# imperatormk/candle-birefnet

Hardware: AMD Instinct MI355X
Metric: images/sec @1024x1024 Swin-L (higher is better)
Workload: dtype f32 storage+accumulate; GEMM operands as two fp16 planes of the power-of-two-scaled operand (22-bit mantissa), 3 fp16 MFMAs/product (fp32-equivalent inside the fp16 range: |GEMM input| < 8190); 1 GPU; BASELINE configs[1]: Swin-L 1024x1024 batch=1 fp32 on 1xMI355X (single-image latency); batch_per_gpu=1, global_batch=1, size=1024, deform_mode=reference_cpu, compute=f32_half2, streams_per_gpu=1, branch_streams_per_gpu=5, inputs=resident in HBM (torch cuda tensors), weights: synthetic seed 42

## Files before the change

### candle_birefnet_amd/csrc/kernels/gemm_split.hip

```cpp
#include "../brn_kernels.h"
#include "gemm_common.h"
#include "gemm_split_stages.h"

namespace brn {

constexpr int SPLIT_LD = 40;

template <int BM, int BN, int WM, int WN, int MODE, int NP, bool H = false>
__global__ void __launch_bounds__(WM* WN * 64) gemm_split_kernel(const GemmParams p) {
    static_assert(!H || NP == 2, "fp16 planes come in pairs");
    constexpr int SLD = SPLIT_LD;
    constexpr int NT = WM * WN * 64;
    constexpr int RPP = NT / 8;
    constexpr int PA = BM / RPP;
    constexpr int WRPP = NT / 4;
    constexpr int PB = BN / WRPP;
    constexpr int WTM = BM / WM, WTN = BN / WN, TM = WTM / 32, TN = WTN / 32;
    static_assert(PA >= 1 && PB >= 1 && TM >= 1 && TN >= 1, "tile too small for the thread count");

    constexpr int SMEM_MAIN = NP * (BM + BN) * SLD * 2, SMEM_EPI = WM * WN * EPI_WAVE_FLOATS * 4;
    __shared__ __attribute__((aligned(16))) char smem_raw[SMEM_MAIN > SMEM_EPI ? SMEM_MAIN : SMEM_EPI];
    __bf16* smem = reinterpret_cast<__bf16*>(smem_raw);
    __bf16* As = smem;
    __bf16* Bs = smem + NP * BM * SLD;

    const int tid = threadIdx.x, lane = tid & 63, wave = tid >> 6;
    const int wm = wave / WN, wn = wave % WN;
    const TileSlice ts = tile_slice<BM, BN>(p, BK);
    const int slice = ts.slice, m0 = ts.m0, n0 = ts.n0, kt0 = ts.kt0, nk = ts.nk;

    const int kq = tid & 7, lrow = tid >> 3;
    long a_base[PA];
    int a_iy[PA], a_ix[PA];
    bool a_ok[PA];
#pragma unroll
    for (int i = 0; i < PA; ++i) gather_row_init<MODE>(p, m0 + lrow + i * RPP, a_ok[i], a_base[i], a_iy[i], a_ix[i]);
    const int wc = tid & 3, wrow = tid >> 2;
    const long wrow_stride = (long)p.K * NP;
    const __bf16* wsrc = reinterpret_cast<const __bf16*>(p.Wp) + (long)(n0 + wrow) * wrow_stride + wc * 8;

    f32x4 ra[2][PA];
    bf16x8 rb[2][NP][PB];
    unsigned am[2][PA];
    constexpr bool DEFORM = MODE == GEMM_DEFORM_NHWC;
    f32x4 rc[DEFORM ? PA : 1][4];
    int rk = 0;
    DeformLoader<PA, 8> dl;
    if constexpr (DEFORM) dl.init(p, m0, lrow, RPP, kq, lane);

    auto gload = [&](int kt, f32x4 (&qa)[PA], bf16x8 (&qb)[NP][PB], unsigned (&qm)[PA]) {
        const int k0 = kt * BK;
#pragma unroll
        for (int pl = 0; pl < NP; ++pl)
#pragma unroll
            for (int i = 0; i < PB; ++i)
                qb[pl][i] = *reinterpret_cast<const bf16x8*>(wsrc + (long)i * WRPP * wrow_stride + (long)kt * (NP * 32) + pl * 32);
        if constexpr (DEFORM) {
            rk = k0;
            dl.template issue<0, PA>(p, k0, rc);
        } else {
            gather_rows_load<MODE>(&p, k0, kq, a_ok, a_base, a_iy, a_ix, qa, qm);
        }
    };
    auto lds_store = [&](const f32x4 (&qa)[PA], const bf16x8 (&qb)[NP][PB], const unsigned (&qm)[PA]) {
#pragma unroll
        for (int i = 0; i < PA; ++i) {
            auto at = [&](int pl) { return As + (pl * BM + lrow + i * RPP) * SLD + kq * 4; };
            if constexpr (DEFORM) stage_a_row<NP, H>(dl.finish(p, rk, i, rc[i]), 0xffffffffu, false, p.a_scale, at);
            else stage_a_row<NP, H>(qa[i], qm[i], true, p.a_scale, at);
        }
        stage_w_planes<NP, PB>(qb, [&](int pl, int i) { return Bs + (pl * BN + wrow + i * WRPP) * SLD + wc * 8; });
    };

    f32x16 acc[TM][TN];
#pragma unroll
    for (int i = 0; i < TM; ++i)
#pragma unroll
        for (int j = 0; j < TN; ++j)
#pragma unroll
            for (int r = 0; r < 16; ++r) acc[i][j][r] = 0.f;

    const __bf16* a_frag = As + (wm * WTM + (lane & 31)) * SLD + (lane >> 5) * 8;
    const __bf16* b_frag = Bs + (wn * WTN + (lane & 31)) * SLD + (lane >> 5) * 8;

    auto compute = [&]() {
#pragma unroll
        for (int ks = 0; ks < 2; ++ks) {
            bf16x8 af[NP][TM], bf[NP][TN];
#pragma unroll
            for (int pl = 0; pl < NP; ++pl) {
#pragma unroll
                for (int i = 0; i < TM; ++i) af[pl][i] = *reinterpret_cast<const bf16x8*>(a_frag + (pl * BM + i * 32) * SLD + ks * 16);
#pragma unroll
                for (int j = 0; j < TN; ++j) bf[pl][j] = *reinterpret_cast<const bf16x8*>(b_frag + (pl * BN + j * 32) * SLD + ks * 16);
            }
            plane_products<NP, H, false>(af, bf, acc);
        }
    };

    if constexpr (DEFORM) {
        if (kt0 < nk) {
            gload(kt0, ra[0], rb[0], am[0]);
            lds_store(ra[0], rb[0], am[0]);
        }
        __syncthreads();
        for (int kt = kt0; kt < nk; ++kt) {
            if (kt + 1 < nk) gload(kt + 1, ra[0], rb[0], am[0]);
            compute();
            __syncthreads();
            if (kt + 1 < nk) {
                lds_store(ra[0], rb[0], am[0]);
                __syncthreads();
            }
        }
    } else {
    if (kt0 < nk) {
        gload(kt0, ra[0], rb[0], am[0]);
        if (kt0 + 1 < nk) gload(kt0 + 1, ra[1], rb[1], am[1]);
        lds_store(ra[0], rb[0], am[0]);
    }
    __syncthreads();
#define BRN_SPLIT_STEP(KT, CUR, NXT)                                  \
    {                                                                 \
        if ((KT) + 2 < nk) gload((KT) + 2, ra[CUR], rb[CUR], am[CUR]);         \
        compute();                                                    \
        __syncthreads();                                              \
        if ((KT) + 1 < nk) {                                          \
            lds_store(ra[NXT], rb[NXT], am[NXT]);            \
            __syncthreads();                                          \
        }                                                             \
    }
    for (int kt = kt0; kt < nk; kt += 2) {
        BRN_SPLIT_STEP(kt, 0, 1)
        if (kt + 1 < nk) BRN_SPLIT_STEP(kt + 1, 1, 0)
    }
#undef BRN_SPLIT_STEP
    }
    gemm_epilogue<TM, TN, WTM, WTN>(p, acc, m0, n0, wm, wn, lane, slice, reinterpret_cast<float*>(smem_raw) + wave * EPI_WAVE_FLOATS);
}

template <int MODE, int NP, int KS, bool DIAG, bool APL, bool H = false>
__global__ void __launch_bounds__(512) __attribute__((amdgpu_waves_per_eu(MODE == GEMM_DEFORM_NHWC && NP == 2 ? 4 : 1)))
gemm_split_ws_kernel(const GemmParams p) {
    using L = WsLayout<NP, KS, APL>;
    constexpr int BM = L::BM, BN = L::BN, WTM = L::WTM, WTN = L::WTN, TM = 2, TN = 2;
    static_assert(!APL || ((NP == 2 || NP == 3) && MODE == GEMM_DENSE), "the P input layout is the NP-plane split of a dense A");
    static_assert(!H || NP == 2, "fp16 planes come in pairs");
    static_assert(L::NBUF == 2, "the producers stage one tile ahead of the consumers; a tile's first fragments are read after the step's barrier");
    constexpr int SLD = L::ROW, KSTEPS = L::KSTEPS, NBUF = L::NBUF, AQ = L::AQ, RPP = L::RPP, PA = L::PA, WQ = L::WQ, WRPP = L::WRPP, PB = L::PB;
    constexpr int APAD = L::APAD, AREG = L::AREG, BUF = L::BUF, EP_LD = L::EP_LD;
    __shared__ __attribute__((aligned(16))) char smem_raw[L::SMEM];
    __bf16* smem = reinterpret_cast<__bf16*>(smem_raw);

    const int tid = threadIdx.x, lane = tid & 63, wave = tid >> 6;
    const int abl = DIAG ? p.abl : 0;
    const bool producer = wave >= 4;
    const TileSlice ts = tile_slice<BM, BN>(p, KS);
    const int slice = ts.slice, m0 = ts.m0, n0 = ts.n0, kt0 = ts.kt0, nk = ts.nk;
    const int nt = nk > kt0 ? nk - kt0 : 0;

    const WsTrace<DIAG> tr(p);
    tr.start(tid);
    f32x16 acc[TM][TN];
    if (producer) {
        const int pt = tid - 256;
        const int kq = pt % AQ, lrow = pt / AQ;
        long a_base[PA];
        int a_iy[PA], a_ix[PA];
        bool a_ok[PA];
        int p_lds[PA];
#pragma unroll
        for (int i = 0; i < PA; ++i) {
            p_lds[i] = 0;
            if (APL) {
                const int q = i * 256 + pt, row = q / (4 * NP), c = q - row * (4 * NP);
                p_lds[i] = ((c >> 2) * BM + row) * SLD + (c >> 2) * APAD + ((c & 3) ^ L::swz_key(row)) * 8;
            }
            gather_row_init<MODE>(p, m0 + lrow + i * RPP, a_ok[i], a_base[i], a_iy[i], a_ix[i]);
        }
        const int wc = pt % WQ, wrow = pt / WQ;
        const int a_sw = ((kq >> 1) ^ L::swz_key(lrow)) * 8 + (kq & 1) * 4;
        const int w_sw = (wc ^ L::swz_key(wrow)) * 8;
        const long wrow_stride = (long)p.K * NP;
        constexpr bool BUFA = MODE == GEMM_DENSE;
        constexpr bool BUFC = MODE == GEMM_CONV_NHWC;
        const int conv_b0 = BUFC ? min(m0, p.M - 1) / (p.Hout * p.Wout) : 0;
        const bool bufc_ok = BUFC && (double)p.Hin * p.Win * p.lda * 8.0 < 2147483648.0;
        __amdgpu_buffer_rsrc_t rsrc_a = BUFC
            ? __builtin_amdgcn_make_buffer_rsrc(const_cast<float*>(p.A + (long)conv_b0 * p.Hin * p.Win * p.lda + p.a_coff), 0, 0x7fffffff, 0x00020000)
            : __builtin_amdgcn_make_buffer_rsrc(const_cast<float*>(p.A + (long)m0 * p.lda), 0, (int)min((long)(p.M - m0) * p.lda * 4, 0x7fffffffL), 0x00020000);
        int conv_pix[PA];
#pragma unroll
        for (int i = 0; i < PA; ++i) {
            conv_pix[i] = 0;
            if (BUFC) {
                const int m = m0 + lrow + i * RPP, hw = p.Hout * p.Wout;
                const int bq = a_ok[i] ? m / hw - conv_b0 : 0;
                conv_pix[i] = (((bq * p.Hin + a_iy[i]) * p.Win + a_ix[i]) * p.lda + kq * 4) * 4;
            }
        }
        __amdgpu_buffer_rsrc_t rsrc_w = __builtin_amdgcn_make_buffer_rsrc(const_cast<__bf16*>(reinterpret_cast<const __bf16*>(p.Wp) + (long)n0 * wrow_stride), 0,
                                                                          0x7fffffff, 0x00020000);
        unsigned voff_a[PA], voff_w[PB];
#pragma unroll
        for (int i = 0; i < PA; ++i) {
            if (APL) { const int q = i * 256 + pt, row = q / (4 * NP), c = q - row * (4 * NP); voff_a[i] = (unsigned)((row * p.lda + c * 4) * 4); }
            else voff_a[i] = (unsigned)(((lrow + i * RPP) * p.lda + kq * 4) * 4);
        }
#pragma unroll
        for (int i = 0; i < PB; ++i) voff_w[i] = (unsigned)(((long)(wrow + i * WRPP) * wrow_stride + wc * 8) * 2);
        f32x4 ra[2][PA];
        bf16x8 rb[2][NP][PB];
        unsigned am[2][PA];
        auto wload = [&](int kt, bf16x8 (&qb)[NP][PB]) {
            const int wk = (KS == 32 ? kt * (NP * 32) : (kt >> 1) * (NP * 32) + (kt & 1) * 16) * 2;
#pragma unroll
            for (int pl = 0; pl < NP; ++pl)
#pragma unroll
                for (int i = 0; i < PB; ++i)
                    qb[pl][i] = __builtin_bit_cast(bf16x8, __builtin_amdgcn_raw_buffer_load_b128(rsrc_w, voff_w[i], wk + pl * 64, 0));
        };
        auto gload = [&](int t, f32x4 (&qa)[PA], bf16x8 (&qb)[NP][PB], unsigned (&qm)[PA]) {
            const int k0 = (kt0 + t) * KS;
            wload(kt0 + t, qb);
            if (BUFA) {
#pragma unroll
                for (int i = 0; i < PA; ++i) {
                    qa[i] = __builtin_bit_cast(f32x4, __builtin_amdgcn_raw_buffer_load_b128(rsrc_a, voff_a[i], APL ? (kt0 + t) * (64 * NP) : k0 * 4, 0));
                    qm[i] = 0xffffffffu;
                }
                return;
            }
            const ConvTap tp = conv_tap(p, k0);
            const int dy = tp.ky * p.dil, dx = tp.kx * p.dil;
            if (bufc_ok) {
                const int tap_off = ((dy * p.Win + dx) * p.lda + tp.ci0) * 4;
#pragma unroll
                for (int i = 0; i < PA; ++i) {
                    const int iy = a_iy[i] + dy, ix = a_ix[i] + dx;
                    const bool ok = a_ok[i] && (unsigned)iy < (unsigned)p.Hin && (unsigned)ix < (unsigned)p.Win;
                    qa[i] = __builtin_bit_cast(f32x4, __builtin_amdgcn_raw_buffer_load_b128(rsrc_a, ok ? (unsigned)(conv_pix[i] + tap_off) : 0x80000000u, 0, 0));
                    qm[i] = 0xffffffffu;
                }
                return;
            }
#pragma unroll
            for (int i = 0; i < PA; ++i) {
                const int iy = a_iy[i] + dy, ix = a_ix[i] + dx;
                const bool ok = a_ok[i] && (unsigned)iy < (unsigned)p.Hin && (unsigned)ix < (unsigned)p.Win;
                const long off = ok ? a_base[i] + ((long)iy * p.Win + ix) * p.lda + tp.ci0 : (long)p.a_coff;
                qa[i] = load4_masked(p.A + off + kq * 4, ok, qm[i]);
            }
        };
        auto w_store = [&](int t, const bf16x8 (&qb)[NP][PB]) {
            __bf16* Bs = smem + (t % NBUF) * BUF + AREG;
            stage_w_planes<NP, PB>(qb, [&](int pl, int i) { return Bs + (pl * BN + wrow + i * WRPP) * SLD + w_sw; });
        };
        auto lds_store = [&](int t, const f32x4 (&qa)[PA], const bf16x8 (&qb)[NP][PB], const unsigned (&qm)[PA]) {
            __bf16* As = smem + (t % NBUF) * BUF;
            if (APL) {
#pragma unroll
                for (int i = 0; i < PA; ++i) {
                    const u32x4 bits = __builtin_bit_cast(u32x4, qa[i]) & qm[i];
                    *reinterpret_cast<u32x4*>(As + p_lds[i]) = bits;
                }
            } else {
#pragma unroll
                for (int i = 0; i < PA; ++i)
                    stage_a_row<NP, H>(qa[i], qm[i], !(BUFA || (BUFC && bufc_ok)), p.a_scale, [&](int pl) { return As + (pl * BM + lrow + i * RPP) * SLD + a_sw; });
            }
            w_store(t, qb);
        };
        if constexpr (MODE == GEMM_DEFORM_NHWC) {
        static_assert(!APL && !DIAG && NBUF == 2 && PA % 2 == 0, "the deformable producer: plain A, the 2-deep ring, rows in two halves");
        constexpr int HR = PA / 2;
        DeformLoader<PA, AQ> dl;
        dl.init(p, m0, lrow, RPP, kq, lane);
        f32x4 rc[PA][4];
        auto a_store = [&](int t, int i, const f32x4 v) {
            __bf16* As = smem + (t % NBUF) * BUF;
            stage_a_row<NP, H>(v, 0xffffffffu, false, p.a_scale, [&](int pl) { return As + (pl * BM + lrow + i * RPP) * SLD + a_sw; });
            __builtin_amdgcn_sched_barrier(0);
        };
        if (nt > 0) { wload(kt0, rb[0]); dl.template issue<0, PA>(p, kt0 * KS, rc); }
        if (nt > 0) {
#pragma unroll
            for (int i = 0; i < PA; ++i) a_store(0, i, dl.finish(p, kt0 * KS, i, rc[i]));
            w_store(0, rb[0]);
        }
        if (nt > 1) { dl.template issue<0, PA>(p, (kt0 + 1) * KS, rc); wload(kt0 + 1, rb[0]); }
        __syncthreads();
        for (int t = 0; t < nt; ++t) {
            const int u = t + 1;
            if (u < nt) {
                const int k0 = (kt0 + u) * KS;
#pragma unroll
                for (int i = 0; i < HR; ++i) a_store(u, i, dl.finish(p, k0, i, rc[i]));
                if (u + 1 < nt) dl.template issue<0, HR>(p, k0 + KS, rc);
#pragma unroll
                for (int i = HR; i < PA; ++i) a_store(u, i, dl.finish(p, k0, i, rc[i]));
                if (u + 1 < nt) dl.template issue<HR, PA>(p, k0 + KS, rc);
                w_store(u, rb[0]);
                if (u + 1 < nt) wload(kt0 + u + 1, rb[0]);
            }
            __syncthreads();
        }
        } else {
        if (nt > 0) gload(0, ra[0], rb[0], am[0]);
        if (nt > 1) gload(1, ra[1], rb[1], am[1]);
        if (nt > 0 && !(abl & 2)) lds_store(0, ra[0], rb[0], am[0]);
        if (nt > 2) gload(2, ra[0], rb[0], am[0]);
        tr.cycles(tid == 256, 8 + 3);
        __syncthreads();
#define BRN_PROD_STEP(T, SET)                                                                      \
        {                                                                                          \
            tr.cycles(tid == 256 && (T) < 24, 16 + (T) * 4 + 0);                                   \
            tr.drain_loads();                                                                      \
            tr.cycles(tid == 256 && (T) < 24, 16 + (T) * 4 + 3);                                   \
            if ((T) + 1 < nt) {                                                                \
                if (!(abl & 2)) lds_store((T) + 1, ra[SET], rb[SET], am[SET]);                 \
                tr.cycles(tid == 256 && (T) < 24, 16 + (T) * 4 + 1);                               \
                if ((T) + 3 < nt && !(abl & 1)) gload((T) + 3, ra[SET], rb[SET], am[SET]); \
            }                                                                                      \
            tr.cycles(tid == 256 && (T) < 24, 16 + (T) * 4 + 2);                                   \
            if (!(abl & 16)) __syncthreads();                                                      \
        }
        for (int t = 0; t < nt; t += 2) {
            BRN_PROD_STEP(t, 1)
            if (t + 1 < nt) BRN_PROD_STEP(t + 1, 0)
        }
#undef BRN_PROD_STEP
        }
        tr.cycles(tid == 256, 8 + 4);
        tr.wall(tid == 256, 8 + 5);
    } else if constexpr (KS == 32 && NP == 2 && !DIAG) {
    f32x4 acc4[4][4];
#pragma unroll
    for (int i = 0; i < 4; ++i)
#pragma unroll
        for (int j = 0; j < 4; ++j) acc4[i][j] = zero4();
    const int wm = wave >> 1, wn = wave & 1;
    const int r16 = lane & 15, kc = lane >> 4;
    const int fch = (kc ^ L::swz_key(r16)) * 8;
    const int a_row = (wm * WTM + r16) * SLD + fch, b_row = AREG + (wn * WTN + r16) * SLD + fch;
    auto read_a = [&](int t, int half, bf16x8 (&af)[NP][2]) {
        const __bf16* buf = smem + (t % NBUF) * BUF;
#pragma unroll
        for (int pl = 0; pl < NP; ++pl)
#pragma unroll
            for (int i = 0; i < 2; ++i) af[pl][i] = *reinterpret_cast<const bf16x8*>(buf + a_row + (pl * BM + (half * 2 + i) * 16) * SLD + pl * APAD);
    };
    auto read_b = [&](int t, int half, bf16x8 (&bf)[NP][2]) {
        const __bf16* buf = smem + (t % NBUF) * BUF;
#pragma unroll
        for (int pl = 0; pl < NP; ++pl)
#pragma unroll
            for (int j = 0; j < 2; ++j) bf[pl][j] = *reinterpret_cast<const bf16x8*>(buf + b_row + (pl * BN + (half * 2 + j) * 16) * SLD);
    };
    bf16x8 fa0[NP][2], fa1[NP][2], fb0[NP][2], fb1[NP][2];
    __syncthreads();
    if (nt > 0) { read_a(0, 0, fa0); read_b(0, 0, fb0); }
    for (int t = 0; t < nt; ++t) {
        read_a(t, 1, fa1);
        read_b(t, 1, fb1);
        plane_products<NP, H, true>(fa0, fb0, acc4, 0, 0);
        plane_products<NP, H, true>(fa1, fb0, acc4, 2, 0);
        plane_products<NP, H, true>(fa0, fb1, acc4, 0, 2);
        plane_products<NP, H, true>(fa1, fb1, acc4, 2, 2);
        __syncthreads();
        if (t + 1 < nt) { read_a(t + 1, 0, fa0); read_b(t + 1, 0, fb0); }
    }
    float* ctile = reinterpret_cast<float*>(smem_raw);
#pragma unroll
    for (int i = 0; i < 4; ++i)
#pragma unroll
        for (int j = 0; j < 4; ++j)
            *reinterpret_cast<f32x4*>(ctile + (wm * WTM + i * 16 + r16) * EP_LD + wn * WTN + j * 16 + 4 * kc) = acc4[i][j];
    } else {
#pragma unroll
    for (int i = 0; i < TM; ++i)
#pragma unroll
        for (int j = 0; j < TN; ++j)
#pragma unroll
            for (int r = 0; r < 16; ++r) acc[i][j][r] = 0.f;
    const int wm = wave >> 1, wn = wave & 1;
    const int fkey = L::swz_key(lane & 31);
    const int a_row = (wm * WTM + (lane & 31)) * SLD, b_row = AREG + (wn * WTN + (lane & 31)) * SLD;
    int f_chunk[KSTEPS];
#pragma unroll
    for (int ks = 0; ks < KSTEPS; ++ks) f_chunk[ks] = (((lane >> 5) + 2 * ks) ^ fkey) * 8;
    auto read_frags = [&](int t, int ks, bf16x8 (&af)[NP][TM], bf16x8 (&bf)[NP][TN]) {
        const __bf16* buf = smem + (t % NBUF) * BUF;
#pragma unroll
        for (int pl = 0; pl < NP; ++pl) {
#pragma unroll
            for (int i = 0; i < TM; ++i) af[pl][i] = *reinterpret_cast<const bf16x8*>(buf + a_row + (pl * BM + i * 32) * SLD + pl * APAD + f_chunk[ks]);
#pragma unroll
            for (int j = 0; j < TN; ++j) bf[pl][j] = *reinterpret_cast<const bf16x8*>(buf + b_row + (pl * BN + j * 32) * SLD + f_chunk[ks]);
        }
    };
    bf16x8 fa0[NP][TM], fb0[NP][TN], fa1[NP][TM], fb1[NP][TN];
    __syncthreads();
    tr.cycles(tid == 0, 3);
    if (nt > 0 && !(abl & 4)) read_frags(0, 0, fa0, fb0);
    for (int t = 0; t < nt; ++t) {
        tr.cycles(tid == 0 && t < 24, 128 + t * 4 + 0);
        if (!(abl & 4)) {
            if (KSTEPS == 2) {
                read_frags(t, 1, fa1, fb1);
                plane_products<NP, H, true>(fa0, fb0, acc);
                plane_products<NP, H, true>(fa1, fb1, acc);
            } else {
                plane_products<NP, H, true>(fa0, fb0, acc);
            }
        }
        tr.cycles(tid == 0 && t < 24, 128 + t * 4 + 1);
        if (!(abl & 16)) __syncthreads();
        if (t + 1 < nt && !(abl & 4)) read_frags(t + 1, 0, fa0, fb0);
    }
    tr.cycles(tid == 0, 4);
    float* ctile = reinterpret_cast<float*>(smem_raw);
    {
        const int row = lane & 31, h4 = (lane >> 5) * 4;
#pragma unroll
        for (int i = 0; i < TM; ++i)
#pragma unroll
            for (int j = 0; j < TN; ++j)
#pragma unroll
                for (int g = 0; g < 4; ++g) {
                    const f32x4 v = {acc[i][j][4 * g], acc[i][j][4 * g + 1], acc[i][j][4 * g + 2], acc[i][j][4 * g + 3]};
                    *reinterpret_cast<f32x4*>(ctile + (wm * WTM + i * 32 + row) * EP_LD + wn * WTN + j * 32 + 8 * g + h4) = v;
                }
    }
    }
    __syncthreads();
    gemm_epilogue_tile<BM, BN, EP_LD>(p, reinterpret_cast<const float*>(smem_raw), m0, n0, tid, slice);
    tr.cycles(tid == 0, 5);
    tr.wall(tid == 0, 6);
}

template <int NP, int KS, bool H>
static hipError_t launch_split_ws_ks(const GemmParams& p, dim3 grid, hipStream_t s) {
    const dim3 block(512);
    if (p.a_planes) {
        if constexpr (NP == 2 && KS == 32) {
            if (p.mode != GEMM_DENSE || p.a_planes != NP) return hipErrorInvalidValue;
#ifdef BRN_DIAG_BUILD
            if constexpr (!H)
                if (p.abl || p.trace) { hipLaunchKernelGGL((gemm_split_ws_kernel<GEMM_DENSE, 2, 32, true, true>), grid, block, 0, s, p); return hipGetLastError(); }
#endif
            hipLaunchKernelGGL((gemm_split_ws_kernel<GEMM_DENSE, 2, 32, false, true, H>), grid, block, 0, s, p);
            return hipGetLastError();
        }
        return hipErrorInvalidValue;
    }
#ifdef BRN_DIAG_BUILD
    if constexpr (!H)
        if (p.mode == GEMM_DENSE && KS == 32 && (p.abl || p.trace)) { hipLaunchKernelGGL((gemm_split_ws_kernel<GEMM_DENSE, NP, 32, true, false>), grid, block, 0, s, p); return hipGetLastError(); }
#endif
    if (p.mode == GEMM_DENSE) hipLaunchKernelGGL((gemm_split_ws_kernel<GEMM_DENSE, NP, KS, false, false, H>), grid, block, 0, s, p);
    else if (p.mode == GEMM_CONV_NHWC) hipLaunchKernelGGL((gemm_split_ws_kernel<GEMM_CONV_NHWC, NP, KS, false, false, H>), grid, block, 0, s, p);
    else if (p.mode == GEMM_DEFORM_NHWC) {
        if constexpr (NP >= 2 && KS == 32) hipLaunchKernelGGL((gemm_split_ws_kernel<GEMM_DEFORM_NHWC, NP, 32, false, false, H>), grid, block, 0, s, p);
        else return hipErrorInvalidValue;
    }
    else return hipErrorInvalidValue;
    return hipGetLastError();
}
template <int NP>
static hipError_t launch_split_ws(const GemmParams& p, hipStream_t s) {
    const int tiles = ((p.M + 127) / 128) * ((p.N + 127) / 128) * p.splitk;
    const dim3 grid(tiles);
    if (p.h2) {
        if constexpr (NP == 2) return launch_split_ws_ks<2, 32, true>(p, grid, s);
        else return hipErrorInvalidValue;
    }
    if constexpr (NP == 3)
        if (tiles > 256 && !(p.abl || p.trace) && p.mode != GEMM_DEFORM_NHWC) return launch_split_ws_ks<3, 16, false>(p, grid, s);
    return launch_split_ws_ks<NP, 32, false>(p, grid, s);
}

template <int BM, int BN, int WM, int WN, int NP, bool H>
static hipError_t launch_split_cfg(const GemmParams& p, hipStream_t s) {
    const int tiles = ((p.M + BM - 1) / BM) * ((p.N + BN - 1) / BN) * p.splitk;
    dim3 grid(tiles), block(WM * WN * 64);
    if (p.mode == GEMM_DENSE) hipLaunchKernelGGL((gemm_split_kernel<BM, BN, WM, WN, GEMM_DENSE, NP, H>), grid, block, 0, s, p);
    else if (p.mode == GEMM_CONV_NHWC) hipLaunchKernelGGL((gemm_split_kernel<BM, BN, WM, WN, GEMM_CONV_NHWC, NP, H>), grid, block, 0, s, p);
    else if (p.mode == GEMM_DEFORM_NHWC) {
        if constexpr (NP >= 2 && BM == 64 && BN == 64) hipLaunchKernelGGL((gemm_split_kernel<64, 64, WM, WN, GEMM_DEFORM_NHWC, NP, H>), grid, block, 0, s, p);
        else return hipErrorInvalidValue;
    }
    else return hipErrorInvalidValue;
    return hipGetLastError();
}
template <int NP, bool H>
static hipError_t launch_split_tile(const GemmParams& p, int cfg, hipStream_t s) {
    if (cfg == 1) return launch_split_cfg<128, 64, 2, 2, NP, H>(p, s);
    return launch_split_cfg<64, 64, 2, 2, NP, H>(p, s);
}

template <int NP>
static hipError_t launch_split_np(const GemmParams& p, int cfg, hipStream_t s) {
    if (gemm_split_is_ws(cfg)) return launch_split_ws<NP>(p, s);
    if (p.h2) {
        if constexpr (NP == 2) return launch_split_tile<2, true>(p, cfg, s);
        else return hipErrorInvalidValue;
    }
    return launch_split_tile<NP, false>(p, cfg, s);
}
hipError_t launch_gemm_split(const GemmParams& p, int cfg, hipStream_t s) {
    if (p.planes == 3) return launch_split_np<3>(p, cfg, s);
    if (p.planes == 2) return launch_split_np<2>(p, cfg, s);
#ifdef BRN_DIAG_BUILD
    return launch_split_np<1>(p, cfg, s);
#else
    return hipErrorInvalidValue;
#endif
}

}
```

Before: 98.11 images/s.

## Add halo-tiled 3x3 conv GEMM kernel reusing staged input across taps

Adds a dedicated kernel for stride-1 same-padding 3x3 NHWC convolutions with two operand planes. Each block stages an 8x16 output tile plus a one-pixel halo of input channels into shared memory once per 32-channel chunk and reuses it for all nine taps, instead of re-gathering im2col rows per tap. Weight fragments are prefetched two taps ahead and shuffled with ds_bpermute, with double-buffered A staging. Eligible convs are routed to it ahead of the generic split GEMM; it risks lower occupancy from the larger shared-memory footprint and edge tiles wasting work on small feature maps.

```diff
diff --git a/candle_birefnet_amd/csrc/kernels/conv_halo_geometry.h b/candle_birefnet_amd/csrc/kernels/conv_halo_geometry.h
--- /dev/null
+++ b/candle_birefnet_amd/csrc/kernels/conv_halo_geometry.h
@@ -0,0 +1,43 @@
+#pragma once
+
+#if defined(__HIP__)
+#define BRN_HALO_HD __host__ __device__
+#else
+#define BRN_HALO_HD
+#endif
+
+namespace brn {
+
+constexpr int HALO_TH = 8, HALO_TW = 16, HALO_BM = HALO_TH * HALO_TW, HALO_BN = 64;
+constexpr int HALO_H = HALO_TH + 2, HALO_W = HALO_TW + 2, HALO_PIXELS = HALO_H * HALO_W;
+constexpr int HALO_CONV_MODE = 1;
+
+struct ConvHaloTile { int b, y0, x0; };
+
+BRN_HALO_HD inline int conv_halo_tiles_y(int H) { return (H + HALO_TH - 1) / HALO_TH; }
+BRN_HALO_HD inline int conv_halo_tiles_x(int W) { return (W + HALO_TW - 1) / HALO_TW; }
+BRN_HALO_HD inline int conv_halo_tiles(int images, int H, int W) { return images * conv_halo_tiles_y(H) * conv_halo_tiles_x(W); }
+BRN_HALO_HD inline ConvHaloTile conv_halo_tile(int H, int W, int tile) {
+    const int tx = conv_halo_tiles_x(W), per_image = conv_halo_tiles_y(H) * tx;
+    const int b = tile / per_image, r = tile - b * per_image;
+    const int ty = r / tx;
+    return ConvHaloTile{b, ty * HALO_TH, (r - ty * tx) * HALO_TW};
+}
+BRN_HALO_HD inline int conv_halo_row(int H, int W, const ConvHaloTile& t, int r) {
+    const int y = t.y0 + r / HALO_TW, x = t.x0 + r % HALO_TW;
+    return (y < H && x < W) ? (t.b * H + y) * W + x : -1;
+}
+BRN_HALO_HD inline int conv_halo_chunks_per_slice(int Cin, int splitk) { return (Cin / 32 + splitk - 1) / splitk; }
+
+template <class P>
+inline bool conv_halo_eligible(const P& p) {
+    const bool conv_two_planes = p.mode == HALO_CONV_MODE && p.planes == 2 && p.Wp != nullptr && !p.a_planes && !p.c_planes && !p.c_bf16;
+    const bool three_by_three_same = p.kh == 3 && p.kw == 3 && p.stride == 1 && p.dil == 1 && p.pad == 1 && p.Hout == p.Hin && p.Wout == p.Win;
+    if (!conv_two_planes || !three_by_three_same || p.Hin <= 0 || p.Win <= 0 || p.Cin <= 0) return false;
+    const bool whole_chunks = p.Cin % 32 == 0 && p.K == 9 * p.Cin && ((p.lda | p.a_coff) & 3) == 0 && p.a_coff + p.Cin <= p.lda;
+    const bool whole_images = p.M > 0 && p.M % (p.Hout * p.Wout) == 0;
+    const bool offsets_fit = (double)p.Hin * p.Win * p.lda * 4.0 < 2147483648.0 && (double)HALO_BN * p.K * 4.0 < 2147483648.0;
+    return whole_chunks && whole_images && offsets_fit && p.splitk >= 1;
+}
+
+}
diff --git a/candle_birefnet_amd/csrc/kernels/gemm_conv_halo.h b/candle_birefnet_amd/csrc/kernels/gemm_conv_halo.h
--- /dev/null
+++ b/candle_birefnet_amd/csrc/kernels/gemm_conv_halo.h
@@ -0,0 +1,167 @@
+#pragma once
+#include <type_traits>
+#include "../brn_kernels.h"
+#include "conv_halo_geometry.h"
+#include "gemm_common.h"
+#include "gemm_split_stages.h"
+
+namespace brn {
+
+struct HaloLayout {
+    static constexpr int NPIX = 192;
+    static constexpr int GROUP = NPIX * 16, PAIR_PAD = 64;
+    static constexpr int PLANE = 4 * GROUP + PAIR_PAD, BUF = 2 * PLANE;
+    static constexpr int EP_LD = HALO_BN + 4;
+    static constexpr int SMEM_MAIN = 2 * BUF, SMEM_EPI = HALO_BM * EP_LD * 4, SMEM = SMEM_MAIN > SMEM_EPI ? SMEM_MAIN : SMEM_EPI;
+    static_assert(NPIX >= HALO_PIXELS && NPIX % 16 == 0 && PLANE % 16 == 0, "fragment reads are 16-byte aligned and conflict-free");
+    static __device__ __forceinline__ int group_off(int g) { return g * GROUP + (g >> 1) * PAIR_PAD; }
+};
+
+template <bool H>
+__global__ void __launch_bounds__(256) conv_halo_kernel(const GemmParams p) {
+    using L = HaloLayout;
+    constexpr int NP = 2, PA = (HALO_PIXELS * 8 + 255) / 256;
+    static_assert(HALO_TW == 16 && HALO_TH == 8 && HALO_BN == 64, "2 x 2 waves of 4 x 2 blocks of 16 x 16");
+    static_assert((256 / 8) * PA <= L::NPIX, "every staged piece has a pixel slot");
+    __shared__ __attribute__((aligned(16))) char smem[L::SMEM];
+
+    const int tid = threadIdx.x, lane = tid & 63, wave = tid >> 6;
+    const int wm = wave >> 1, wn = wave & 1;
+    const int r16 = lane & 15, kc = lane >> 4;
+
+    const int Hm = p.Hout, Wm = p.Wout;
+    const int tiles_n = (p.N + HALO_BN - 1) / HALO_BN;
+    const int ntiles = conv_halo_tiles(p.M / (Hm * Wm), Hm, Wm) * tiles_n;
+    const int swz = xcd_remap();
+    const int slice = swz / ntiles, t = swz - slice * ntiles;
+    const int tile_m = t / tiles_n, n0 = (t - tile_m * tiles_n) * HALO_BN;
+    const ConvHaloTile tl = conv_halo_tile(Hm, Wm, tile_m);
+    const int nch = p.Cin / 32, per = conv_halo_chunks_per_slice(p.Cin, p.splitk);
+    const int c0 = slice * per, c1 = min(nch, c0 + per);
+
+    const __amdgpu_buffer_rsrc_t rsrc_a =
+        __builtin_amdgcn_make_buffer_rsrc(const_cast<float*>(p.A + (long)tl.b * p.Hin * p.Win * p.lda + p.a_coff), 0, 0x7fffffff, 0x00020000);
+    const int kq = tid & 7;
+    unsigned voff_a[PA];
+#pragma unroll
+    for (int i = 0; i < PA; ++i) {
+        const int hp = (tid >> 3) + 32 * i, hy = hp / HALO_W, hx = hp - hy * HALO_W;
+        const int y = tl.y0 - 1 + hy, x = tl.x0 - 1 + hx;
+        const bool ok = hp < HALO_PIXELS && (unsigned)y < (unsigned)p.Hin && (unsigned)x < (unsigned)p.Win;
+        voff_a[i] = ok ? (unsigned)(((y * p.Win + x) * p.lda + kq * 4) * 4) : 0x80000000u;
+    }
+    const int a_st = L::group_off(kq >> 1) + (tid >> 3) * 16 + (kq & 1) * 8;
+    const long wrow_stride = (long)p.K * NP;
+    const __amdgpu_buffer_rsrc_t rsrc_w = __builtin_amdgcn_make_buffer_rsrc(
+        const_cast<__bf16*>(reinterpret_cast<const __bf16*>(p.Wp) + (long)n0 * wrow_stride), 0, 0x7fffffff, 0x00020000);
+    unsigned voff_w[2];
+#pragma unroll
+    for (int j = 0; j < 2; ++j) voff_w[j] = (unsigned)(((long)(wn * 32 + j * 16 + (lane >> 2)) * wrow_stride + (lane & 3) * 8) * 2);
+    const int w_src = (r16 * 4 + kc) * 4;
+    const int a_rd = L::group_off(kc) + (wm * 4 * HALO_W + r16) * 16;
+
+    f32x4 ra[PA];
+    u32x4 wraw[NP][2];
+    bf16x8 wb[2][NP][2];
+    f32x4 acc[4][2];
+#pragma unroll
+    for (int i = 0; i < 4; ++i)
+#pragma unroll
+        for (int j = 0; j < 2; ++j) acc[i][j] = zero4();
+
+    auto aload = [&](int c) {
+#pragma unroll
+        for (int i = 0; i < PA; ++i) ra[i] = __builtin_bit_cast(f32x4, __builtin_amdgcn_raw_buffer_load_b128(rsrc_a, voff_a[i], c * 128, 0));
+    };
+    auto astore = [&](int buf) {
+        char* dst = smem + buf * L::BUF + a_st;
+#pragma unroll
+        for (int i = 0; i < PA; ++i) stage_a_row<NP, H>(ra[i], 0xffffffffu, false, p.a_scale, [&](int pl) { return dst + pl * L::PLANE + i * 512; });
+    };
+    auto wload = [&](int c, int tap) {
+        if (tap >= 9) { tap -= 9; ++c; }
+        if (c >= c1) return;
+        const int wk = (tap * nch + c) * (NP * 64);
+#pragma unroll
+        for (int pl = 0; pl < NP; ++pl)
+#pragma unroll
+            for (int j = 0; j < 2; ++j) wraw[pl][j] = __builtin_bit_cast(u32x4, __builtin_amdgcn_raw_buffer_load_b128(rsrc_w, voff_w[j], wk + pl * 64, 0));
+    };
+    auto wpermute = [&](bf16x8 (&q)[NP][2]) {
+#pragma unroll
+        for (int pl = 0; pl < NP; ++pl)
+#pragma unroll
+            for (int j = 0; j < 2; ++j) {
+                u32x4 v;
+#pragma unroll
+                for (int e = 0; e < 4; ++e) v[e] = (unsigned)__builtin_amdgcn_ds_bpermute(w_src, (int)wraw[pl][j][e]);
+                q[pl][j] = __builtin_bit_cast(bf16x8, v);
+            }
+    };
+    auto chunk = [&](int c, int buf, auto par) {
+        constexpr int PAR = decltype(par)::value;
+        const bool more = c + 1 < c1;
+        if (more) aload(c + 1);
+        const char* src = smem + buf * L::BUF + a_rd;
+#pragma unroll
+        for (int tap = 0; tap < 9; ++tap) {
+            const int cur = (tap + PAR) & 1, ky = tap / 3, kx = tap - ky * 3;
+            if (tap < 8 || more) wpermute(wb[cur ^ 1]);
+            wload(c, tap + 2);
+            __builtin_amdgcn_sched_barrier(0);
+#pragma unroll
+            for (int half = 0; half < 2; ++half) {
+                bf16x8 af[NP][2];
+#pragma unroll
+                for (int pl = 0; pl < NP; ++pl)
+#pragma unroll
+                    for (int i = 0; i < 2; ++i)
+                        af[pl][i] = *reinterpret_cast<const bf16x8*>(src + pl * L::PLANE + ((half * 2 + i + ky) * HALO_W + kx) * 16);
+                plane_products<NP, H, true>(af, wb[cur], acc, half * 2, 0);
+            }
+        }
+        if (more) astore(buf ^ 1);
+        __syncthreads();
+    };
+
+    if (c0 < c1) {
+        aload(c0);
+        wload(c0, 0);
+        astore(0);
+        wpermute(wb[0]);
+        wload(c0, 1);
+        __syncthreads();
+    }
+    for (int c = c0; c < c1; c += 2) {
+        chunk(c, 0, std::integral_constant<int, 0>{});
+        if (c + 1 < c1) chunk(c + 1, 1, std::integral_constant<int, 1>{});
+    }
+
+    float* ctile = reinterpret_cast<float*>(smem);
+#pragma unroll
+    for (int i = 0; i < 4; ++i)
+#pragma unroll
+        for (int j = 0; j < 2; ++j)
+            *reinterpret_cast<f32x4*>(ctile + (wm * 64 + i * 16 + r16) * L::EP_LD + wn * 32 + j * 16 + 4 * kc) = acc[i][j];
+    __syncthreads();
+    const int c4 = (tid & 15) * 4, n = n0 + c4;
+    if (n >= p.N) return;
+    const EpiCols cols = epilogue_cols(p, slice, n);
+#pragma unroll 2
+    for (int ps = 0; ps < HALO_BM / 16; ++ps) {
+        const int row = ps * 16 + (tid >> 4);
+        const int m = conv_halo_row(Hm, Wm, tl, row);
+        if (m < 0) continue;
+        epilogue_row<false, false>(p, cols, m, n, *reinterpret_cast<const f32x4*>(ctile + row * L::EP_LD + c4));
+    }
+}
+
+template <bool H>
+static hipError_t launch_conv_halo(const GemmParams& p, hipStream_t s) {
+    static_assert(HALO_CONV_MODE == GEMM_CONV_NHWC, "conv_halo_geometry.h names the mode by value");
+    const int tiles = conv_halo_tiles(p.M / (p.Hout * p.Wout), p.Hout, p.Wout) * ((p.N + HALO_BN - 1) / HALO_BN) * p.splitk;
+    hipLaunchKernelGGL((conv_halo_kernel<H>), dim3(tiles), dim3(256), 0, s, p);
+    return hipGetLastError();
+}
+
+}
diff --git a/candle_birefnet_amd/csrc/kernels/gemm_split.hip b/candle_birefnet_amd/csrc/kernels/gemm_split.hip
--- a/candle_birefnet_amd/csrc/kernels/gemm_split.hip
+++ b/candle_birefnet_amd/csrc/kernels/gemm_split.hip
@@ -1,6 +1,7 @@
 #include "../brn_kernels.h"
 #include "gemm_common.h"
 #include "gemm_split_stages.h"
+#include "gemm_conv_halo.h"
 
 namespace brn {
 
@@ -502,6 +503,8 @@
 template <int NP>
 static hipError_t launch_split_np(const GemmParams& p, int cfg, hipStream_t s) {
     if (gemm_split_is_ws(cfg)) return launch_split_ws<NP>(p, s);
+    if constexpr (NP == 2)
+        if (conv_halo_eligible(p)) return p.h2 ? launch_conv_halo<true>(p, s) : launch_conv_halo<false>(p, s);
     if (p.h2) {
         if constexpr (NP == 2) return launch_split_tile<2, true>(p, cfg, s);
         else return hipErrorInvalidValue;
```

Result: faster. 99.85 images/s, median of 6 (+1.8%).
